# microsoft/ptgnn

Measured on NVIDIA H100. Metric: edges/sec per GNN layer, higher is better.
Workload: dtype f32

## Files before the change

### ptgnn_b200/csrc/plan.cu

```cuda
#include "common.cuh"

namespace ptgnn {

constexpr int SCAN_THREADS = 256;
constexpr int SCAN_ITEMS = 16;
constexpr int SCAN_CHUNK = SCAN_THREADS * SCAN_ITEMS;

__device__ __forceinline__ int warp_inclusive_scan(int v) {
    const int lane = threadIdx.x & 31;
#pragma unroll
    for (int o = 1; o < 32; o <<= 1) {
        int n = __shfl_up_sync(0xffffffffu, v, o);
        if (lane >= o) v += n;
    }
    return v;
}

template <int THREADS>
__device__ __forceinline__ int block_exclusive_scan(int v, int *total) {
    __shared__ int warp_sums[THREADS / 32];
    __shared__ int block_total;
    const int lane = threadIdx.x & 31, warp = threadIdx.x >> 5;
    int incl = warp_inclusive_scan(v);
    if (lane == 31) warp_sums[warp] = incl;
// ... 157 lines not shown
        }
    }
    __syncthreads();
#pragma unroll
    for (int r = 0; r < SORT_ROUNDS; ++r) {
        const bool valid = digit[r] < RADIX;
        const unsigned peers = __match_any_sync(0xffffffffu, digit[r]);
        int dst = 0;
        if (valid) dst = warp_hist[warp][digit[r]] + __popc(peers & ((1u << lane) - 1u));
        __syncwarp();
        if (valid && lane == __ffs(peers) - 1) warp_hist[warp][digit[r]] += __popc(peers);
        __syncwarp();
        if (valid) {
            keys_out[dst] = key[r];
            vals_out[dst] = val[r];
        }
    }
}

__global__ void __launch_bounds__(256) finalize_plan_kernel(const __grid_constant__ TypeOffsets toff, int64_t num_edges,
                                                            const int32_t *__restrict__ perm,
                                                            const int32_t *__restrict__ src32,
                                                            int32_t *__restrict__ pos, int32_t *__restrict__ src_sorted,
                                                            uint8_t *__restrict__ etype_sorted) {
    for (int64_t j = (int64_t)blockIdx.x * blockDim.x + threadIdx.x; j < num_edges;
         j += (int64_t)gridDim.x * blockDim.x) {
        const int32_t e = perm[j];
        pos[e] = (int32_t)j;
        src_sorted[j] = src32[e];
        etype_sorted[j] = (uint8_t)type_of_edge(toff.off, toff.num_types, e);
    }
}

struct PlanWs {
    size_t deg, scan_sums, keys_a, keys_b, vals_a, vals_b, hist, hist_sums, total;
};
static PlanWs plan_ws_layout(int64_t N, int64_t E) {
    PlanWs w{};
    const int64_t nblk = ceil_div(E > 0 ? E : 1, SORT_CHUNK);
    size_t o = 0;
    auto add = [&](size_t cnt) { size_t at = o; o += ws_slice(cnt, 4); return at; };
    w.deg = add((size_t)N + 1);
    w.scan_sums = add(scan_workspace_elems(N + 1));
    w.keys_a = add((size_t)E + 1);
    w.keys_b = add((size_t)E + 1);
    w.vals_a = add((size_t)E + 1);
    w.vals_b = add((size_t)E + 1);
    w.hist = add((size_t)RADIX * nblk);
    w.hist_sums = add(scan_workspace_elems((int64_t)RADIX * nblk));
    w.total = o;
    return w;
}

static int sort_edges_by_key(const int32_t *keys_in, int key_bits, int64_t E, int32_t *perm, char *ws, const PlanWs &L,
                             cudaStream_t st, const int32_t **sorted_keys = nullptr) {
    const int64_t nblk = ceil_div(E, SORT_CHUNK);
    int32_t *keys[2] = {reinterpret_cast<int32_t *>(ws + L.keys_a), reinterpret_cast<int32_t *>(ws + L.keys_b)};
    int32_t *vals[2] = {reinterpret_cast<int32_t *>(ws + L.vals_a), reinterpret_cast<int32_t *>(ws + L.vals_b)};
    int32_t *hist = reinterpret_cast<int32_t *>(ws + L.hist);
    int32_t *hist_sums = reinterpret_cast<int32_t *>(ws + L.hist_sums);
    const int passes = (key_bits + RADIX_BITS - 1) / RADIX_BITS;
    const int32_t *kin = keys_in;
    const int32_t *vin = nullptr;
    for (int p = 0; p < passes; ++p) {
        int32_t *kout = keys[p & 1];
        int32_t *vout = (p == passes - 1) ? perm : vals[p & 1];
        {
            TimedScope timed__(PTGNN_KERNEL_PLAN, st);
            radix_hist_kernel<<<(unsigned)nblk, SORT_THREADS, 0, st>>>(kin, E, p * RADIX_BITS, hist);
        }
        PTGNN_LAUNCHED();
        int rc = exclusive_scan_i32(hist, hist, (int64_t)RADIX * nblk, hist_sums, nullptr, st);
        if (rc) return rc;
        {
            TimedScope timed__(PTGNN_KERNEL_PLAN, st);
            radix_scatter_kernel<<<(unsigned)nblk, SORT_THREADS, 0, st>>>(kin, vin, E, p * RADIX_BITS, p == 0, hist, kout,
                                                                      vout);
        }
        PTGNN_LAUNCHED();
        kin = kout;
        vin = vout;
    }
    if (sorted_keys) *sorted_keys = kin;
    return PTGNN_OK;
}
static int bits_for(int64_t n) {
    int bits = 1;
    while (bits < 31 && ((int64_t)1 << bits) < n) ++bits;
    return bits;
}
static int sort_edges_by_target(const int32_t *tgt32, int64_t N, int64_t E, int32_t *perm, char *ws, const PlanWs &L,
                                cudaStream_t st) {
    return sort_edges_by_key(tgt32, bits_for(N), E, perm, ws, L, st);
}

__global__ void __launch_bounds__(256) block_keys_kernel(const __grid_constant__ TypeOffsets toff, int64_t num_edges,
                                                         const int32_t *__restrict__ tgt32, int B, int32_t *__restrict__ keys,
                                                         int32_t *__restrict__ group_count) {
    for (int64_t e = (int64_t)blockIdx.x * blockDim.x + threadIdx.x; e < num_edges; e += (int64_t)gridDim.x * blockDim.x) {
        const int t = type_of_edge(toff.off, toff.num_types, e);
        const int v = tgt32[e];
        const int blk = v / B, tl = v - blk * B;
        keys[e] = (blk * toff.num_types + t) * B + tl;
        atomicAdd(&group_count[(int64_t)blk * toff.num_types + t], 1);
    }
}
__global__ void __launch_bounds__(256) block_finalize_kernel(int64_t num_edges, int B, const int32_t *__restrict__ perm,
                                                             const int32_t *__restrict__ sorted_keys,
                                                             const int32_t *__restrict__ src32, int32_t *__restrict__ src_f,
                                                             uint8_t *__restrict__ tl_f) {
    for (int64_t j = (int64_t)blockIdx.x * blockDim.x + threadIdx.x; j < num_edges; j += (int64_t)gridDim.x * blockDim.x) {
        src_f[j] = src32[perm[j]];
        tl_f[j] = (uint8_t)(sorted_keys[j] % B);
    }
}
struct BlockPlanWs { size_t keys, perm, scan_sums, plan, total; };
static BlockPlanWs block_plan_ws_layout(int64_t N, int64_t E, int T, int B) {
    BlockPlanWs w{};
    const int64_t nblk = ceil_div(N > 0 ? N : 1, B), groups = nblk * (T > 0 ? T : 1) + 1;
    size_t o = 0;
    auto add = [&](size_t cnt) { size_t at = o; o += ws_slice(cnt, 4); return at; };
    w.keys = add((size_t)E + 1);
    w.perm = add((size_t)E + 1);
    w.scan_sums = add(scan_workspace_elems(groups));
    w.plan = o; o += plan_ws_layout(N, E).total;
    w.total = o;
    return w;
}

}

using namespace ptgnn;

extern "C" size_t ptgnn_b200_plan_workspace_bytes(int64_t num_nodes, int64_t num_edges) {
    if (num_nodes < 0 || num_edges < 0) return 0;
    return plan_ws_layout(num_nodes, num_edges).total;
}

static int plan_build_phases(int phases, int64_t num_nodes, int64_t num_source_nodes, int32_t num_types,
                             const int64_t *const *src_ptrs, const int64_t *const *tgt_ptrs, const int64_t *counts, int32_t *row_ptr,
                             int32_t *perm, int32_t *pos, int32_t *src_sorted, uint8_t *etype_sorted, int32_t *src32, int32_t *tgt32,
                             int32_t *status, void *workspace, size_t workspace_bytes, void *stream) {
    cudaStream_t st = static_cast<cudaStream_t>(stream);
    PTGNN_CHECK_ARG(num_nodes >= 0 && num_nodes < INT32_MAX, "plan_build: num_nodes=%lld out of range", (long long)num_nodes);
    if (num_source_nodes <= 0) num_source_nodes = num_nodes;
    PTGNN_CHECK_ARG(num_source_nodes < INT32_MAX, "plan_build: num_source_nodes out of range");
    PTGNN_CHECK_ARG(num_types >= 0 && num_types <= PTGNN_MAX_EDGE_TYPES, "plan_build: num_types=%d (max %d)", num_types,
                    PTGNN_MAX_EDGE_TYPES);
    PTGNN_CHECK_ARG(row_ptr && status, "plan_build: null row_ptr/status");
    EdgeTables tabs{};
    TypeOffsets toff{};
    tabs.num_types = toff.num_types = num_types;
    int64_t E = 0;
    for (int t = 0; t < num_types; ++t) {
        PTGNN_CHECK_ARG(counts[t] >= 0, "plan_build: negative edge count for type %d", t);
        PTGNN_CHECK_ARG(counts[t] == 0 || !(phases & 1) || (src_ptrs[t] && tgt_ptrs[t]), "plan_build: null edge list for type %d", t);
        tabs.src[t] = (phases & 1) ? src_ptrs[t] : nullptr;
        tabs.tgt[t] = (phases & 1) ? tgt_ptrs[t] : nullptr;
        tabs.off[t] = E;
        toff.off[t] = (int32_t)E;
        E += counts[t];
        PTGNN_CHECK_ARG(E < INT32_MAX, "plan_build: more than 2^31-1 edges");
    }
    tabs.off[num_types] = E;
    toff.off[num_types] = (int32_t)E;
    for (int t = num_types + 1; t <= PTGNN_MAX_EDGE_TYPES; ++t) { tabs.off[t] = E; toff.off[t] = (int32_t)E; }

    const PlanWs L = plan_ws_layout(num_nodes, E);
    PTGNN_CHECK_WORKSPACE("plan_build", workspace, workspace_bytes, L.total);
    char *ws = static_cast<char *>(workspace);
    int32_t *deg = reinterpret_cast<int32_t *>(ws + L.deg);

    const unsigned grid = (unsigned)(ceil_div(E > 0 ? E : 1, 256) < 132 * 16 ? ceil_div(E > 0 ? E : 1, 256) : 132 * 16);
    int rc = PTGNN_OK;
    if (phases & 1) {
        PTGNN_CUDA(cudaMemsetAsync(status, 0, sizeof(int32_t), st));
        PTGNN_CUDA(cudaMemsetAsync(deg, 0, sizeof(int32_t) * (size_t)(num_nodes + 1), st));
        if (E == 0) {
// ... 14 lines not shown
    PTGNN_CHECK_ARG(perm && pos && src_sorted && etype_sorted && src32 && tgt32, "plan_build: null output array");
    rc = sort_edges_by_target(tgt32, num_nodes, E, perm, ws, L, st);
    if (rc) return rc;
    {
        TimedScope timed__(PTGNN_KERNEL_PLAN, st);
        finalize_plan_kernel<<<grid, 256, 0, st>>>(toff, E, perm, src32, pos, src_sorted, etype_sorted);
    }
    PTGNN_LAUNCHED();
    return PTGNN_OK;
}

extern "C" int ptgnn_b200_plan_build(int64_t num_nodes, int64_t num_source_nodes, int32_t num_types,
                                     const int64_t *const *src_ptrs, const int64_t *const *tgt_ptrs, const int64_t *counts,
                                     int32_t *row_ptr, int32_t *perm, int32_t *pos, int32_t *src_sorted, uint8_t *etype_sorted,
                                     int32_t *src32, int32_t *tgt32, int32_t *status, void *workspace, size_t workspace_bytes,
                                     void *stream) {
    return plan_build_phases(3, num_nodes, num_source_nodes, num_types, src_ptrs, tgt_ptrs, counts, row_ptr, perm, pos, src_sorted,
                             etype_sorted, src32, tgt32, status, workspace, workspace_bytes, stream);
}
extern "C" int ptgnn_b200_plan_convert(int64_t num_nodes, int64_t num_source_nodes, int32_t num_types,
                                       const int64_t *const *src_ptrs, const int64_t *const *tgt_ptrs, const int64_t *counts,
                                       int32_t *row_ptr, int32_t *src32, int32_t *tgt32, int32_t *status, void *workspace,
                                       size_t workspace_bytes, void *stream) {
    return plan_build_phases(1, num_nodes, num_source_nodes, num_types, src_ptrs, tgt_ptrs, counts, row_ptr, nullptr, nullptr, nullptr,
                             nullptr, src32, tgt32, status, workspace, workspace_bytes, stream);
}
extern "C" int ptgnn_b200_plan_sort(int64_t num_nodes, int32_t num_types, const int64_t *counts, int32_t *perm, int32_t *pos,
                                    int32_t *src_sorted, uint8_t *etype_sorted, const int32_t *src32, const int32_t *tgt32,
                                    void *workspace, size_t workspace_bytes, void *stream) {
    int32_t dummy_status = 0;
    return plan_build_phases(2, num_nodes, num_nodes, num_types, nullptr, nullptr, counts, &dummy_status , perm, pos,
                             src_sorted, etype_sorted, const_cast<int32_t *>(src32), const_cast<int32_t *>(tgt32), &dummy_status, workspace,
                             workspace_bytes, stream);
}

extern "C" size_t ptgnn_b200_block_plan_workspace_bytes(int64_t num_nodes, int64_t num_edges, int32_t num_types,
                                                        int32_t block_targets) {
    if (num_nodes < 0 || num_edges < 0 || num_types < 0 || block_targets <= 0) return 0;
    return block_plan_ws_layout(num_nodes, num_edges, num_types, block_targets).total;
}

extern "C" int ptgnn_b200_block_plan_build(int64_t num_nodes, int32_t num_types, const int64_t *type_off,
                                           const int32_t *src32, const int32_t *tgt32, int32_t block_targets,
                                           int32_t *group_off, int32_t *src_f, uint8_t *tl_f, void *workspace,
                                           size_t workspace_bytes, void *stream) {
    cudaStream_t st = static_cast<cudaStream_t>(stream);
    const int B = block_targets, T = num_types;
    PTGNN_CHECK_ARG(num_nodes >= 0 && num_nodes < INT32_MAX, "block_plan_build: num_nodes out of range");
    PTGNN_CHECK_ARG(T > 0 && T <= PTGNN_MAX_EDGE_TYPES && type_off, "block_plan_build: bad num_types=%d", T);
    PTGNN_CHECK_ARG(B >= 8 && B <= 256, "block_plan_build: block_targets=%d must be in [8, 256]", B);
    const int64_t E = type_off[T];
    PTGNN_CHECK_ARG(E >= 0 && E < INT32_MAX, "block_plan_build: edge count out of range");
    const int64_t nblk = ceil_div(num_nodes, B), groups = nblk * T;
    PTGNN_CHECK_ARG(nblk * T * B < ((int64_t)1 << 31), "block_plan_build: %lld blocks x %d types x %d targets overflow the 31-bit sort key",
                    (long long)nblk, T, B);
    PTGNN_CHECK_ARG(group_off, "block_plan_build: null group_off");
    const BlockPlanWs L = block_plan_ws_layout(num_nodes, E, T, B);
    PTGNN_CHECK_WORKSPACE("block_plan_build", workspace, workspace_bytes, L.total);
    PTGNN_CUDA(cudaMemsetAsync(group_off, 0, sizeof(int32_t) * (size_t)(groups + 1), st));
    if (E == 0 || num_nodes == 0) return PTGNN_OK;
    PTGNN_CHECK_ARG(src32 && tgt32 && src_f && tl_f, "block_plan_build: null edge array");
    char *ws = static_cast<char *>(workspace);
    int32_t *keys = reinterpret_cast<int32_t *>(ws + L.keys), *perm = reinterpret_cast<int32_t *>(ws + L.perm);
    TypeOffsets toff{};
    toff.num_types = T;
    for (int t = 0; t <= PTGNN_MAX_EDGE_TYPES; ++t) toff.off[t] = (int32_t)type_off[t < T ? t : T];
    const unsigned grid = (unsigned)(ceil_div(E, 256) < 132 * 16 ? ceil_div(E, 256) : 132 * 16);
    {
        TimedScope timed__(PTGNN_KERNEL_PLAN, st);
        block_keys_kernel<<<grid, 256, 0, st>>>(toff, E, tgt32, B, keys, group_off);
    }
    PTGNN_LAUNCHED();
    int rc = exclusive_scan_i32(group_off, group_off, groups + 1, reinterpret_cast<int32_t *>(ws + L.scan_sums), nullptr, st);
    if (rc) return rc;
    const int32_t *sorted_keys = nullptr;
    rc = sort_edges_by_key(keys, bits_for(nblk * T * B), E, perm, ws + L.plan, plan_ws_layout(num_nodes, E), st, &sorted_keys);
    if (rc) return rc;
    {
        TimedScope timed__(PTGNN_KERNEL_PLAN, st);
        block_finalize_kernel<<<grid, 256, 0, st>>>(E, B, perm, sorted_keys, src32, src_f, tl_f);
    }
    PTGNN_LAUNCHED();
    return PTGNN_OK;
}
```

### ptgnn_b200/csrc/fused_mp.cu

```cuda
#include "fused_mp.cuh"

#include <cuda_bf16.h>
#include <cuda_fp16.h>
#include <float.h>
#include <stdlib.h>

#include <type_traits>

#include "tc_common.cuh"

namespace ptgnn {
namespace fused {

using tc::mbar_arrive;
using tc::mbar_init;
using tc::mbar_wait;

constexpr int NUM_THREADS = 16 * 32;
constexpr int GATHER_WARP0 = 8, GATHER_THREADS = 64;
constexpr int SCHED_WARP = 10;
constexpr int REDUCER_WARP0 = 12;
constexpr int SCHED_READER_WARPS = 8 + 2 + 4;
constexpr int NUM_SLOTS = 3, LOOKAHEAD = 2;
constexpr int SLOT_BYTES = 32768;
constexpr int RING_BYTES = NUM_SLOTS * SLOT_BYTES;
constexpr int META_RING = 8;
constexpr int SCHED_RING = 4;
constexpr int PRODUCER_REGS = 56, CONSUMER_REGS = 184, REDUCER_REGS = 88;
static_assert(PRODUCER_REGS + 2 * CONSUMER_REGS + REDUCER_REGS <= 4 * 128, "register budgets exceed the launch allocation");
constexpr int NMAX = 64;
constexpr int ACC_PITCH = NMAX + 4;
constexpr int ACC_BYTES = kD * ACC_PITCH * 4;
constexpr int RED_BAR_ID = 1;

struct Meta {
    int32_t tloff[128];
    uint32_t endmask[4];
    int32_t n, pad[3];
};
struct Sched {
    int32_t blk, pad[3];
    int32_t off[PTGNN_MAX_EDGE_TYPES + 4];
};
constexpr int ACC_OFF = RING_BYTES;
constexpr int AGG_OFF = RING_BYTES + ACC_BYTES;
__host__ __device__ constexpr int agg_bytes(int B) { return B * kD * 4; }
constexpr int SMEM_TAIL = META_RING * (int)sizeof(Meta) + SCHED_RING * (int)sizeof(Sched) + 256 ;
constexpr int smem_bytes(int B) { return 1024 + RING_BYTES + ACC_BYTES + agg_bytes(B) + SMEM_TAIL; }
static_assert(smem_bytes(kMaxBlockTargets) <= 232448, "shared memory budget");

struct Params {
    const unsigned char *src_rows, *tgt_rows;
    const uint4 *wpack;
    const int32_t *group_off, *src_f;
    const uint8_t *tl_f;
    const int32_t *row_ptr;
    void *out;
    int num_nodes, num_blocks, B, T, reduce, out_mode;
    int32_t *status;
    unsigned long long *trace;
    Epilogue epi;
    EgcEpilogue egc;
};
constexpr int EPI_AGG = 0, EPI_EGC = 1;

__device__ __forceinline__ uint4 ldg_nc_u4(const uint4 *p) {
    uint4 r;
    asm volatile("ld.global.nc.L1::no_allocate.v4.u32 {%0,%1,%2,%3}, [%4];" : "=r"(r.x), "=r"(r.y), "=r"(r.z), "=r"(r.w) : "l"(p));
    return r;
}
__device__ __forceinline__ void named_bar_sync(int id, int threads) { asm volatile("bar.sync %0, %1;" ::"r"(id), "r"(threads) : "memory"); }
__device__ __forceinline__ uint32_t swz(int row, int q) { return (uint32_t)(row * 128 + ((q ^ (row & 7)) << 4)); }

constexpr int TRACE_ROLES = 4, TRACE_CAP = 8192;
__shared__ uint32_t trace_n[TRACE_ROLES];
__device__ __forceinline__ void trace_mark(const Params &p, int tag, uint32_t step) {
    if (p.trace == nullptr || blockIdx.x != 0) return;
    const int tid = (int)threadIdx.x;
    const int role = tid == GATHER_WARP0 * 32 ? 0 : (tid == 0 ? 1 : (tid == 128 ? 2 : (tid == REDUCER_WARP0 * 32 ? 3 : -1)));
    if (role < 0) return;
    const uint32_t n = trace_n[role];
    if (n >= TRACE_CAP) return;
    p.trace[role * TRACE_CAP + n] = ((unsigned long long)clock64() << 24) | ((unsigned long long)(step & 0xFFFFu) << 8) | (unsigned)(tag & 0xFF);
    trace_n[role] = n + 1;
}

struct Step { int blk, t, e, n, seg; };
template <int NSEG>
struct StepGen {
    const Sched *sched;
    uint64_t *sfull, *sempty;
    int T, nmax, lane;
    uint32_t it = 0;
    const Sched *tab = nullptr;
    int blk = -1, t = 0, e = 0, e1 = 0, seg = 0;
    __device__ __forceinline__ int next(Step &s) {
        for (;;) {
            if (tab == nullptr) {
                const uint32_t r = it % SCHED_RING;
                mbar_wait(&sfull[r], (it / SCHED_RING) & 1);
                blk = sched[r].blk;
                if (blk < 0) return 2;
                tab = &sched[r];
                t = -1; e = e1 = 0; seg = 0;
            }
            if (e < e1) {
                s.blk = blk; s.t = t; s.e = e; s.n = min(nmax, e1 - e); s.seg = seg;
                if (++seg == NSEG) { seg = 0; e += nmax; }
                return 0;
            }
            ++t;
            while (t < T && tab->off[t + 1] == tab->off[t]) ++t;
            if (t >= T) {
                tab = nullptr;
                s.blk = blk;
                __syncwarp();
                if (lane == 0) mbar_arrive(&sempty[it % SCHED_RING]);
                ++it;
                return 1;
            }
            e = tab->off[t]; e1 = tab->off[t + 1]; seg = 0;
        }
    }
// ... 363 lines not shown
                    if (lane == 0) m->endmask[c >> 5] = word;
                }
                if (g == 0) m->n = st.n;
                ++sgc;
            };
            auto issue_next = [&]() {
                cur = nxt;
                int idx[NMAX / 8];
#pragma unroll
                for (int i = 0; i < NMAX / 8; ++i) idx[i] = idx_nxt[i];
                finish_meta(cur);
                const uint32_t slot = c_issue % NUM_SLOTS;
                trace_mark(p, 1, c_issue);
                mbar_wait(&x_empty[slot], ((c_issue / NUM_SLOTS) & 1) ^ 1);
                trace_mark(p, 2, c_issue);
                const unsigned char *rows = cur.seg == 0 ? p.src_rows : p.tgt_rows;
                const uint32_t sbase = smem_u32(ring + slot * SLOT_BYTES) + swz(rsub, q);
#pragma unroll
                for (int i = 0; i < NMAX / 8; ++i) {
                    if (idx[i] >= 0) {
                        const unsigned char *src = rows + (size_t)idx[i] * ROW_BYTES + q * 16;
#pragma unroll
                        for (int ti = 0; ti < NT; ++ti)
                            cp_async16(sbase + ti * TILE_BYTES + i * 1024, src + (ti / KCH) * (K * 2) + (ti % KCH) * 128, 16);
                    }
                }
                trace_mark(p, 3, c_issue);
                ++c_issue;
            };
            fetch();
            bool more = has_nxt;
            while (more) {
                const uint32_t slot = c_issue % NUM_SLOTS;
                issue_next();
                asm volatile("cp.async.mbarrier.arrive.noinc.shared::cta.b64 [%0];" ::"r"(smem_u32(&x_full[slot])) : "memory");
                trace_mark(p, 4, c_done);
                mbar_arrive(&x_full[slot]);
                ++c_done;
                fetch();
                more = has_nxt;
            }
            cp_async_wait<0>();
        }
    } else {
        tc::reg_alloc<CONSUMER_REGS>();
        const int eg = warp >> 2, ew = warp & 3;
        const int gq = lane >> 2, tq = lane & 3;
        const int f0 = 64 * eg + 16 * ew + gq;
        StepGen<NSEG> gen{sched, sched_full, sched_empty, T, NMAX, lane};
        uint32_t sg = 0, xs = 0;
        int w_t = -1, w_seg = -1;
        uint32_t wf[NPART][K / 16][4];
        float acc_m[32], acc_c[32];
        auto load_weights = [&](const Step &st) {
            const uint32_t *wp = reinterpret_cast<const uint32_t *>(p.wpack + (size_t)(st.t * NSEG + st.seg) * NPART * (K / 8) * 128);
#pragma unroll
            for (int part = 0; part < NPART; ++part)
#pragma unroll
                for (int ks = 0; ks < K / 16; ++ks)
#pragma unroll
                    for (int i = 0; i < 4; ++i) {
                        const int c4 = (part * (K / 8) + 2 * ks + (i >> 1)), f = f0 + 8 * (i & 1);
                        wf[part][ks][i] = __ldg(wp + ((size_t)c4 * 128 + f) * 4 + tq);
                    }
            w_t = st.t; w_seg = st.seg;
            trace_mark(p, 11, xs);
        };
        auto mma = [&](auto nb_tag, uint32_t slot_addr) {
            constexpr int NB = decltype(nb_tag)::value;
#pragma unroll
            for (int ks = 0; ks < K / 16; ++ks) {
                const int kc = ks >> 2, kk = ks & 3;
                const uint64_t x_hi = tc::make_smem_desc_sw128(slot_addr + kc * TILE_BYTES) + kk * 2;
                const uint64_t x_lo = tc::make_smem_desc_sw128(slot_addr + (KCH + kc) * TILE_BYTES) + kk * 2;
                auto one = [&](float (&dacc)[32], const uint32_t (&a)[4], uint64_t desc) {
                    if (NB == 1) tc::wgmma_16_rs_n16<BF16>(dacc, a, desc);
                    else if (NB == 2) tc::wgmma_16_rs_n32<BF16>(dacc, a, desc);
                    else if (NB == 3) tc::wgmma_16_rs_n48<BF16>(dacc, a, desc);
                    else tc::wgmma_16_rs_n64<BF16>(dacc, a, desc);
                };
                one(acc_m, wf[0][ks], x_hi);
                if (NPROD == 3) {
                    one(acc_c, wf[0][ks], x_lo);
                    one(acc_c, wf[NPART - 1][ks], x_hi);
                }
            }
        };
        Step s, nx;
        int ev = gen.next(s);
        while (ev != 2) {
            if (ev == 0) {
                trace_mark(p, 10, xs);
                if (s.t != w_t || s.seg != w_seg) load_weights(s);
                const uint32_t slot = xs % NUM_SLOTS;
                mbar_wait(&x_full[slot], (xs / NUM_SLOTS) & 1);
                tc::fence_proxy_async_smem();
                trace_mark(p, 12, xs);
                if (tc::warp_uniform(s.seg) == 0) {
#pragma unroll
                    for (int i = 0; i < 32; ++i) { acc_m[i] = 0.0f; acc_c[i] = 0.0f; }
                }
                const uint32_t slot_addr = smem_u32(ring + slot * SLOT_BYTES);
                const int nb = tc::warp_uniform((s.n + 15) >> 4);
                tc::wgmma_fence();
                using std::integral_constant;
                if (nb == 1) mma(integral_constant<int, 1>{}, slot_addr);
                else if (nb == 2) mma(integral_constant<int, 2>{}, slot_addr);
                else if (nb == 3) mma(integral_constant<int, 3>{}, slot_addr);
                else mma(integral_constant<int, 4>{}, slot_addr);
                tc::wgmma_commit();
                trace_mark(p, 13, xs);
                tc::wgmma_wait<0>();
                tc::fence_acc(acc_m);
                if (NPROD == 3) tc::fence_acc(acc_c);
                __syncwarp();
                if (lane == 0) mbar_arrive(&x_empty[slot]);
                trace_mark(p, 14, xs);
                ++xs;
                const int evn = gen.next(nx);
                if (evn == 0 && (nx.t != w_t || nx.seg != w_seg)) load_weights(nx);
                if (s.seg == NSEG - 1) {
                    trace_mark(p, 20, sg);
                    mbar_wait(acc_empty, (sg & 1) ^ 1);
                    trace_mark(p, 21, sg);
#pragma unroll
                    for (int j = 0; j < 8; ++j) {
                        if (8 * j < 16 * nb) {
#pragma unroll
                        for (int h = 0; h < 2; ++h) {
                            float v0 = acc_m[4 * j + 2 * h], v1 = acc_m[4 * j + 2 * h + 1];
                            if (NPROD == 3) {
                                v0 = fmaf(acc_c[4 * j + 2 * h], 1.0f / 2048.0f, v0); v1 = fmaf(acc_c[4 * j + 2 * h + 1], 1.0f / 2048.0f, v1);
                            } else {
                                v0 = __bfloat162float(__float2bfloat16_rn(v0)); v1 = __bfloat162float(__float2bfloat16_rn(v1));
                            }
                            *reinterpret_cast<float2 *>(acc_s + (f0 + 8 * h) * ACC_PITCH + 8 * j + 2 * tq) = make_float2(v0, v1);
                        }
                        }
                    }
                    __syncwarp();
                    if (lane == 0) mbar_arrive(acc_full);
                    trace_mark(p, 22, sg);
                    ++sg;
                }
                s = nx; ev = evn;
                continue;
            }
            ev = gen.next(s);
        }
    }
}

__global__ void __launch_bounds__(256) pack_states_kernel(const float *__restrict__ h, long long rows, int K,
                                                          uint4 *__restrict__ out, int32_t *__restrict__ status) {
    const long long total = rows * (K / 8);
    bool bad = false;
    for (long long i = (long long)blockIdx.x * blockDim.x + threadIdx.x; i < total; i += (long long)gridDim.x * blockDim.x) {
        const long long row = i / (K / 8);
        const int c8 = (int)(i - row * (K / 8));
        const float4 a = ld_stream_f4(reinterpret_cast<const float4 *>(h + row * K + c8 * 8));
        const float4 b = ld_stream_f4(reinterpret_cast<const float4 *>(h + row * K + c8 * 8 + 4));
        const float x[8] = {a.x, a.y, a.z, a.w, b.x, b.y, b.z, b.w};
        __half hi[8], lo[8];
#pragma unroll
        for (int j = 0; j < 8; ++j) bad |= !split_f16(x[j], hi[j], lo[j]);
        uint4 vh, vl;
        vh.x = pack_h2(hi[0], hi[1]); vh.y = pack_h2(hi[2], hi[3]); vh.z = pack_h2(hi[4], hi[5]); vh.w = pack_h2(hi[6], hi[7]);
        vl.x = pack_h2(lo[0], lo[1]); vl.y = pack_h2(lo[2], lo[3]); vl.z = pack_h2(lo[4], lo[5]); vl.w = pack_h2(lo[6], lo[7]);
        uint4 *dst = out + row * (K / 4);
        dst[c8] = vh;
        dst[K / 8 + c8] = vl;
    }
    if (bad && status != nullptr) *reinterpret_cast<volatile int32_t *>(status) = 1;
}

struct WeightSrc {
    const float *w[PTGNN_MAX_EDGE_TYPES];
};
template <int NPROD>
__global__ void __launch_bounds__(256) pack_weights_kernel(const __grid_constant__ WeightSrc src, int num_types, int K, int nseg,
                                                           RowMap rows, uint4 *__restrict__ out, int32_t *__restrict__ status) {
    constexpr int NPART = NPROD == 3 ? 2 : 1;
    const int per_mat = nseg * (K / 8) * 128;
    const long long total = (long long)num_types * per_mat;
    bool bad = false;
    for (long long i = (long long)blockIdx.x * blockDim.x + threadIdx.x; i < total; i += (long long)gridDim.x * blockDim.x) {
        const int t = (int)(i / per_mat);
        int r = (int)(i - (long long)t * per_mat);
        const int seg = r / ((K / 8) * 128);
        r -= seg * (K / 8) * 128;
        const int c4 = r / 128, d = r % 128;
        int srow = d;
        if (rows.bases > 0) {
            const int o = rows.col0 + d / rows.bases, b = d % rows.bases;
            srow = ((o / rows.dh) * rows.bases + b) * rows.dh + o % rows.dh;
        }
        const float *row = src.w[t] + (size_t)srow * (nseg * K) + seg * K + c4 * 8;
        float x[8];
#pragma unroll
        for (int j = 0; j < 8; ++j) x[j] = row[j];
        const size_t base = ((size_t)(t * nseg + seg) * NPART) * (K / 8) * 128;
        if (NPROD == 3) {
            __half hi[8], lo[8];
#pragma unroll
            for (int j = 0; j < 8; ++j) bad |= !split_f16(x[j], hi[j], lo[j]);
            uint4 vh, vl;
            vh.x = pack_h2(hi[0], hi[1]); vh.y = pack_h2(hi[2], hi[3]); vh.z = pack_h2(hi[4], hi[5]); vh.w = pack_h2(hi[6], hi[7]);
            vl.x = pack_h2(lo[0], lo[1]); vl.y = pack_h2(lo[2], lo[3]); vl.z = pack_h2(lo[4], lo[5]); vl.w = pack_h2(lo[6], lo[7]);
            out[base + (size_t)c4 * 128 + d] = vh;
            out[base + (size_t)(K / 8 + c4) * 128 + d] = vl;
        } else {
            uint4 v;
            __nv_bfloat162 p0 = __floats2bfloat162_rn(x[0], x[1]), p1 = __floats2bfloat162_rn(x[2], x[3]);
            __nv_bfloat162 p2 = __floats2bfloat162_rn(x[4], x[5]), p3 = __floats2bfloat162_rn(x[6], x[7]);
            v.x = *reinterpret_cast<uint32_t *>(&p0); v.y = *reinterpret_cast<uint32_t *>(&p1);
            v.z = *reinterpret_cast<uint32_t *>(&p2); v.w = *reinterpret_cast<uint32_t *>(&p3);
            out[base + (size_t)c4 * 128 + d] = v;
        }
    }
    if (bad && status != nullptr) *reinterpret_cast<volatile int32_t *>(status + 1) = 1;
}

bool supported(int nprod, int K, int D, int use_target) {
    (void)use_target;
    if (D != kD) return false;
    if (nprod == 3) return K == 64 || K == 128;
    if (nprod == 1) return K == 64 || K == 128 || K == 256;
    return false;
}
size_t packed_weight_bytes(int nprod, int num_types, int K, int use_target) {
    const int nseg = use_target ? 2 : 1, npart = nprod == 3 ? 2 : 1;
    return ws_slice((size_t)num_types * nseg * npart * (K / 8) * 128, 16);
}
size_t packed_state_bytes(int nprod, int64_t rows, int K) {
    return nprod == 3 ? ws_slice((size_t)rows * K * 4 + 16, 1) : 0;
}
int recommended_block_targets(int64_t num_nodes) {
    if (num_nodes <= 0) return kMaxBlockTargets;
    const int64_t waves = ceil_div(num_nodes, (int64_t)kMaxBlockTargets * 132);
    int64_t B = ceil_div(num_nodes, waves * 132);
    B = (B + 7) / 8 * 8;
    if (B < 8) B = 8;
    if (B > kMaxBlockTargets) B = kMaxBlockTargets;
    return (int)B;
}

int pack_weights(int nprod, int num_types, int K, int use_target, const float *const *weights, void *packed, int32_t *status,
                 cudaStream_t st, RowMap rows) {
    WeightSrc src{};
    for (int t = 0; t < num_types; ++t) src.w[t] = weights[t];
    const int nseg = use_target ? 2 : 1;
    {
        TimedScope timed__(PTGNN_KERNEL_PACK, st);
        if (nprod == 3) pack_weights_kernel<3><<<132, 256, 0, st>>>(src, num_types, K, nseg, rows, static_cast<uint4 *>(packed), status);
        else pack_weights_kernel<1><<<132, 256, 0, st>>>(src, num_types, K, nseg, rows, static_cast<uint4 *>(packed), status);
    }
    PTGNN_LAUNCHED();
    return PTGNN_OK;
}

int pack_states(const float *h, int64_t rows, int K, void *packed, int32_t *status, cudaStream_t st) {
    if (rows <= 0) return PTGNN_OK;
    const int64_t items = rows * (K / 8);
    const unsigned grid = (unsigned)(ceil_div(items, 256) < 132 * 8 ? ceil_div(items, 256) : 132 * 8);
    {
        TimedScope timed__(PTGNN_KERNEL_PACK, st);
        pack_states_kernel<<<grid, 256, 0, st>>>(h, (long long)rows, K, static_cast<uint4 *>(packed), status);
    }
    PTGNN_LAUNCHED();
    return PTGNN_OK;
}

template <int NPROD, int K, int NSEG, int RED, int EPI = EPI_AGG>
static int launch_one(const Params &p, cudaStream_t st) {
    auto kernel = fused_aggregate_kernel<NPROD, K, NSEG, RED, EPI>;
    const int smem = smem_bytes(p.B);
    PTGNN_CUDA(cudaFuncSetAttribute(kernel, cudaFuncAttributeMaxDynamicSharedMemorySize, smem));
    const int sms = sm_count();
    const int grid = p.num_blocks < sms ? p.num_blocks : sms;
    {
        TimedScope timed__(PTGNN_KERNEL_MESSAGE, st);
        kernel<<<grid, NUM_THREADS, smem, st>>>(p);
    }
    PTGNN_LAUNCHED();
    return PTGNN_OK;
// ... 80 lines not shown
```

Before: 1.339 billion.

## Replace global radix sort in block plan with bucket scatter and per-group sort

The block plan build no longer runs a multi-pass global radix sort over composite keys. Instead it counts edges per (block, type) group using warp-aggregated atomics, scans the counts, and scatters packed (target-local, edge-id) items into group buckets. Each bucket is then sorted in place: small groups by a per-warp rank sort in shared memory, large ones by a CTA-wide radix sort. This cuts the number of full-array passes and launches, at the cost of nondeterministic scatter order fixed by the per-group sort, and quadratic work for groups near the size cap.

Result: faster. 1.372 billion (median of 6 runs) (+2.4%).

```diff
diff --git a/ptgnn_b200/csrc/plan.cu b/ptgnn_b200/csrc/plan.cu
--- a/ptgnn_b200/csrc/plan.cu
+++ b/ptgnn_b200/csrc/plan.cu
@@ -233,15 +233,20 @@
     return w;
 }
 
-static int sort_edges_by_key(const int32_t *keys_in, int key_bits, int64_t E, int32_t *perm, char *ws, const PlanWs &L,
-                             cudaStream_t st, const int32_t **sorted_keys = nullptr) {
+static int bits_for(int64_t n) {
+    int bits = 1;
+    while (bits < 31 && ((int64_t)1 << bits) < n) ++bits;
+    return bits;
+}
+static int sort_edges_by_target(const int32_t *tgt32, int64_t N, int64_t E, int32_t *perm, char *ws, const PlanWs &L,
+                                cudaStream_t st) {
     const int64_t nblk = ceil_div(E, SORT_CHUNK);
     int32_t *keys[2] = {reinterpret_cast<int32_t *>(ws + L.keys_a), reinterpret_cast<int32_t *>(ws + L.keys_b)};
     int32_t *vals[2] = {reinterpret_cast<int32_t *>(ws + L.vals_a), reinterpret_cast<int32_t *>(ws + L.vals_b)};
     int32_t *hist = reinterpret_cast<int32_t *>(ws + L.hist);
     int32_t *hist_sums = reinterpret_cast<int32_t *>(ws + L.hist_sums);
-    const int passes = (key_bits + RADIX_BITS - 1) / RADIX_BITS;
-    const int32_t *kin = keys_in;
+    const int passes = (bits_for(N) + RADIX_BITS - 1) / RADIX_BITS;
+    const int32_t *kin = tgt32;
     const int32_t *vin = nullptr;
     for (int p = 0; p < passes; ++p) {
         int32_t *kout = keys[p & 1];
@@ -262,49 +267,173 @@
         kin = kout;
         vin = vout;
     }
-    if (sorted_keys) *sorted_keys = kin;
     return PTGNN_OK;
 }
-static int bits_for(int64_t n) {
-    int bits = 1;
-    while (bits < 31 && ((int64_t)1 << bits) < n) ++bits;
-    return bits;
-}
-static int sort_edges_by_target(const int32_t *tgt32, int64_t N, int64_t E, int32_t *perm, char *ws, const PlanWs &L,
-                                cudaStream_t st) {
-    return sort_edges_by_key(tgt32, bits_for(N), E, perm, ws, L, st);
-}
-
-__global__ void __launch_bounds__(256) block_keys_kernel(const __grid_constant__ TypeOffsets toff, int64_t num_edges,
-                                                         const int32_t *__restrict__ tgt32, int B, int32_t *__restrict__ keys,
-                                                         int32_t *__restrict__ group_count) {
+
+struct EdgeGroup { int64_t g; int tl; };
+__device__ __forceinline__ EdgeGroup edge_group(const TypeOffsets &toff, const int32_t *__restrict__ tgt32, int B, int64_t e) {
+    const int t = type_of_edge(toff.off, toff.num_types, e);
+    const int v = tgt32[e];
+    const int blk = v / B;
+    return {(int64_t)blk * toff.num_types + t, v - blk * B};
+}
+
+__global__ void __launch_bounds__(256) block_count_kernel(const __grid_constant__ TypeOffsets toff, int64_t num_edges,
+                                                          const int32_t *__restrict__ tgt32, int B, int32_t *__restrict__ group_count) {
     for (int64_t e = (int64_t)blockIdx.x * blockDim.x + threadIdx.x; e < num_edges; e += (int64_t)gridDim.x * blockDim.x) {
-        const int t = type_of_edge(toff.off, toff.num_types, e);
-        const int v = tgt32[e];
-        const int blk = v / B, tl = v - blk * B;
-        keys[e] = (blk * toff.num_types + t) * B + tl;
-        atomicAdd(&group_count[(int64_t)blk * toff.num_types + t], 1);
-    }
-}
-__global__ void __launch_bounds__(256) block_finalize_kernel(int64_t num_edges, int B, const int32_t *__restrict__ perm,
-                                                             const int32_t *__restrict__ sorted_keys,
-                                                             const int32_t *__restrict__ src32, int32_t *__restrict__ src_f,
-                                                             uint8_t *__restrict__ tl_f) {
-    for (int64_t j = (int64_t)blockIdx.x * blockDim.x + threadIdx.x; j < num_edges; j += (int64_t)gridDim.x * blockDim.x) {
-        src_f[j] = src32[perm[j]];
-        tl_f[j] = (uint8_t)(sorted_keys[j] % B);
-    }
-}
-struct BlockPlanWs { size_t keys, perm, scan_sums, plan, total; };
+        const int64_t g = edge_group(toff, tgt32, B, e).g;
+        const unsigned peers = __match_any_sync(__activemask(), (unsigned long long)g);
+        if ((threadIdx.x & 31) == __ffs(peers) - 1) atomicAdd(&group_count[g], __popc(peers));
+    }
+}
+
+__global__ void __launch_bounds__(256) block_scatter_kernel(const __grid_constant__ TypeOffsets toff, int64_t num_edges,
+                                                            const int32_t *__restrict__ tgt32, int B,
+                                                            const int32_t *__restrict__ group_off, int32_t *__restrict__ group_count,
+                                                            uint64_t *__restrict__ items) {
+    for (int64_t e = (int64_t)blockIdx.x * blockDim.x + threadIdx.x; e < num_edges; e += (int64_t)gridDim.x * blockDim.x) {
+        const EdgeGroup eg = edge_group(toff, tgt32, B, e);
+        const int lane = threadIdx.x & 31;
+        const unsigned peers = __match_any_sync(__activemask(), (unsigned long long)eg.g);
+        const int leader = __ffs(peers) - 1;
+        int left = 0;
+        if (lane == leader) left = atomicSub(&group_count[eg.g], __popc(peers));
+        left = __shfl_sync(peers, left, leader);
+        const int32_t slot = group_off[eg.g] + left - 1 - __popc(peers & ((1u << lane) - 1u));
+        items[slot] = ((uint64_t)eg.tl << 32) | (uint32_t)e;
+    }
+}
+
+constexpr int GSORT_WARPS = 8;
+constexpr int GSORT_THREADS = GSORT_WARPS * 32;
+constexpr int GSORT_CAP = 512;
+constexpr int GSORT_ILP = 2;
+constexpr int GSORT_RADIX_PASSES = 5;
+
+struct GroupSortSmem {
+    union {
+        uint64_t warp_items[GSORT_WARPS][GSORT_CAP];
+        struct {
+            int bin[256];
+            int warp_cnt[GSORT_WARPS][256];
+        } radix;
+    };
+};
+
+__device__ __forceinline__ void write_group(uint64_t it, int64_t j, const int32_t *__restrict__ src32, int32_t *__restrict__ src_f,
+                                            uint8_t *__restrict__ tl_f) {
+    src_f[j] = src32[(uint32_t)it];
+    tl_f[j] = (uint8_t)(it >> 32);
+}
+
+__device__ __noinline__ void cta_radix_sort_group(GroupSortSmem &sm, uint64_t *__restrict__ items, uint64_t *__restrict__ items_alt, int64_t lo,
+                                     int n, const int32_t *__restrict__ src32, int32_t *__restrict__ src_f, uint8_t *__restrict__ tl_f) {
+    const int tid = threadIdx.x, lane = tid & 31, warp = tid >> 5;
+    const uint64_t *in = items + lo;
+    uint64_t *out = items_alt + lo;
+    for (int p = 0; p < GSORT_RADIX_PASSES; ++p) {
+        const int shift = 8 * p;
+        sm.radix.bin[tid] = 0;
+        __syncthreads();
+        for (int i = tid; i < n; i += GSORT_THREADS) atomicAdd(&sm.radix.bin[(in[i] >> shift) & 255], 1);
+        __syncthreads();
+        int total;
+        sm.radix.bin[tid] = block_exclusive_scan<GSORT_THREADS>(sm.radix.bin[tid], &total);
+        for (int64_t base = 0; base < n; base += GSORT_THREADS) {
+#pragma unroll
+            for (int w = 0; w < GSORT_WARPS; ++w) sm.radix.warp_cnt[w][tid] = 0;
+            __syncthreads();
+            const int64_t i = base + tid;
+            const bool valid = i < n;
+            const uint64_t it = valid ? in[i] : 0;
+            const int d = valid ? (int)((it >> shift) & 255) : 256;
+            const unsigned peers = __match_any_sync(0xffffffffu, d);
+            const int rank = __popc(peers & ((1u << lane) - 1u));
+            if (valid && lane == __ffs(peers) - 1) sm.radix.warp_cnt[warp][d] = __popc(peers);
+            __syncthreads();
+            {
+                int run = sm.radix.bin[tid];
+#pragma unroll
+                for (int w = 0; w < GSORT_WARPS; ++w) {
+                    const int c = sm.radix.warp_cnt[w][tid];
+                    sm.radix.warp_cnt[w][tid] = run;
+                    run += c;
+                }
+                sm.radix.bin[tid] = run;
+            }
+            __syncthreads();
+            if (valid) out[sm.radix.warp_cnt[warp][d] + rank] = it;
+            __syncthreads();
+        }
+        const uint64_t *next_in = out;
+        out = const_cast<uint64_t *>(in);
+        in = next_in;
+    }
+    for (int i = tid; i < n; i += GSORT_THREADS) write_group(in[i], lo + i, src32, src_f, tl_f);
+    __syncthreads();
+}
+
+__global__ void __launch_bounds__(GSORT_THREADS) block_group_sort_kernel(int64_t groups, const int32_t *__restrict__ group_off,
+                                                                         uint64_t *__restrict__ items, uint64_t *__restrict__ items_alt,
+                                                                         const int32_t *__restrict__ src32, int32_t *__restrict__ src_f,
+                                                                         uint8_t *__restrict__ tl_f) {
+    __shared__ GroupSortSmem sm;
+    const int lane = threadIdx.x & 31, warp = threadIdx.x >> 5;
+    const int64_t g0 = (int64_t)blockIdx.x * GSORT_WARPS;
+    if (g0 + warp < groups) {
+        const int64_t lo = group_off[g0 + warp];
+        const int n = group_off[g0 + warp + 1] - (int32_t)lo;
+        if (n <= GSORT_CAP) {
+            uint64_t *s = sm.warp_items[warp];
+            for (int base = 0; base < n; base += 32 * GSORT_ILP) {
+                uint64_t v[GSORT_ILP];
+#pragma unroll
+                for (int q = 0; q < GSORT_ILP; ++q) v[q] = base + q * 32 + lane < n ? items[lo + base + q * 32 + lane] : 0;
+#pragma unroll
+                for (int q = 0; q < GSORT_ILP; ++q)
+                    if (base + q * 32 + lane < n) s[base + q * 32 + lane] = v[q];
+            }
+            __syncwarp();
+            for (int base = 0; base < n; base += 32 * GSORT_ILP) {
+                uint64_t mine[GSORT_ILP];
+                int rank[GSORT_ILP];
+#pragma unroll
+                for (int q = 0; q < GSORT_ILP; ++q) {
+                    mine[q] = base + q * 32 + lane < n ? s[base + q * 32 + lane] : 0;
+                    rank[q] = 0;
+                }
+#pragma unroll 4
+                for (int j = 0; j < n; ++j) {
+                    const uint64_t x = s[j];
+#pragma unroll
+                    for (int q = 0; q < GSORT_ILP; ++q) rank[q] += x < mine[q];
+                }
+#pragma unroll
+                for (int q = 0; q < GSORT_ILP; ++q)
+                    if (base + q * 32 + lane < n) write_group(mine[q], lo + rank[q], src32, src_f, tl_f);
+            }
+        }
+    }
+    for (int w = 0; w < GSORT_WARPS && g0 + w < groups; ++w) {
+        const int64_t lo = group_off[g0 + w];
+        const int n = group_off[g0 + w + 1] - (int32_t)lo;
+        if (n > GSORT_CAP) {
+            __syncthreads();
+            cta_radix_sort_group(sm, items, items_alt, lo, n, src32, src_f, tl_f);
+        }
+    }
+}
+
+struct BlockPlanWs { size_t group_count, scan_sums, items, items_alt, total; };
 static BlockPlanWs block_plan_ws_layout(int64_t N, int64_t E, int T, int B) {
     BlockPlanWs w{};
     const int64_t nblk = ceil_div(N > 0 ? N : 1, B), groups = nblk * (T > 0 ? T : 1) + 1;
     size_t o = 0;
-    auto add = [&](size_t cnt) { size_t at = o; o += ws_slice(cnt, 4); return at; };
-    w.keys = add((size_t)E + 1);
-    w.perm = add((size_t)E + 1);
-    w.scan_sums = add(scan_workspace_elems(groups));
-    w.plan = o; o += plan_ws_layout(N, E).total;
+    auto add = [&](size_t cnt, size_t elt) { size_t at = o; o += ws_slice(cnt, elt); return at; };
+    w.group_count = add((size_t)groups, 4);
+    w.scan_sums = add(scan_workspace_elems(groups), 4);
+    w.items = add((size_t)E + 1, 8);
+    w.items_alt = add((size_t)E + 1, 8);
     w.total = o;
     return w;
 }
@@ -425,33 +554,40 @@
     const int64_t E = type_off[T];
     PTGNN_CHECK_ARG(E >= 0 && E < INT32_MAX, "block_plan_build: edge count out of range");
     const int64_t nblk = ceil_div(num_nodes, B), groups = nblk * T;
-    PTGNN_CHECK_ARG(nblk * T * B < ((int64_t)1 << 31), "block_plan_build: %lld blocks x %d types x %d targets overflow the 31-bit sort key",
+    PTGNN_CHECK_ARG(nblk * T * B < ((int64_t)1 << 31), "block_plan_build: %lld blocks x %d types x %d targets exceed 2^31",
                     (long long)nblk, T, B);
     PTGNN_CHECK_ARG(group_off, "block_plan_build: null group_off");
     const BlockPlanWs L = block_plan_ws_layout(num_nodes, E, T, B);
     PTGNN_CHECK_WORKSPACE("block_plan_build", workspace, workspace_bytes, L.total);
-    PTGNN_CUDA(cudaMemsetAsync(group_off, 0, sizeof(int32_t) * (size_t)(groups + 1), st));
-    if (E == 0 || num_nodes == 0) return PTGNN_OK;
+    if (E == 0 || num_nodes == 0) {
+        PTGNN_CUDA(cudaMemsetAsync(group_off, 0, sizeof(int32_t) * (size_t)(groups + 1), st));
+        return PTGNN_OK;
+    }
     PTGNN_CHECK_ARG(src32 && tgt32 && src_f && tl_f, "block_plan_build: null edge array");
     char *ws = static_cast<char *>(workspace);
-    int32_t *keys = reinterpret_cast<int32_t *>(ws + L.keys), *perm = reinterpret_cast<int32_t *>(ws + L.perm);
+    int32_t *group_count = reinterpret_cast<int32_t *>(ws + L.group_count);
+    uint64_t *items = reinterpret_cast<uint64_t *>(ws + L.items), *items_alt = reinterpret_cast<uint64_t *>(ws + L.items_alt);
     TypeOffsets toff{};
     toff.num_types = T;
     for (int t = 0; t <= PTGNN_MAX_EDGE_TYPES; ++t) toff.off[t] = (int32_t)type_off[t < T ? t : T];
     const unsigned grid = (unsigned)(ceil_div(E, 256) < 132 * 16 ? ceil_div(E, 256) : 132 * 16);
-    {
-        TimedScope timed__(PTGNN_KERNEL_PLAN, st);
-        block_keys_kernel<<<grid, 256, 0, st>>>(toff, E, tgt32, B, keys, group_off);
-    }
-    PTGNN_LAUNCHED();
-    int rc = exclusive_scan_i32(group_off, group_off, groups + 1, reinterpret_cast<int32_t *>(ws + L.scan_sums), nullptr, st);
+    PTGNN_CUDA(cudaMemsetAsync(group_count, 0, sizeof(int32_t) * (size_t)(groups + 1), st));
+    {
+        TimedScope timed__(PTGNN_KERNEL_PLAN, st);
+        block_count_kernel<<<grid, 256, 0, st>>>(toff, E, tgt32, B, group_count);
+    }
+    PTGNN_LAUNCHED();
+    int rc = exclusive_scan_i32(group_count, group_off, groups + 1, reinterpret_cast<int32_t *>(ws + L.scan_sums), nullptr, st);
     if (rc) return rc;
-    const int32_t *sorted_keys = nullptr;
-    rc = sort_edges_by_key(keys, bits_for(nblk * T * B), E, perm, ws + L.plan, plan_ws_layout(num_nodes, E), st, &sorted_keys);
-    if (rc) return rc;
-    {
-        TimedScope timed__(PTGNN_KERNEL_PLAN, st);
-        block_finalize_kernel<<<grid, 256, 0, st>>>(E, B, perm, sorted_keys, src32, src_f, tl_f);
+    {
+        TimedScope timed__(PTGNN_KERNEL_PLAN, st);
+        block_scatter_kernel<<<grid, 256, 0, st>>>(toff, E, tgt32, B, group_off, group_count, items);
+    }
+    PTGNN_LAUNCHED();
+    {
+        TimedScope timed__(PTGNN_KERNEL_PLAN, st);
+        block_group_sort_kernel<<<(unsigned)ceil_div(groups, GSORT_WARPS), GSORT_THREADS, 0, st>>>(groups, group_off, items, items_alt,
+                                                                                                  src32, src_f, tl_f);
     }
     PTGNN_LAUNCHED();
     return PTGNN_OK;
```

## Pack weights in per-lane fragment order and stagger reloads across warpgroups

Applied to the files above, without the earlier changes.

The weight packing kernel now writes the A-operand register fragments so that each consumer lane fetches one contiguous uint4 per k-step. This replaces four strided 32-bit loads per k-step with a single coalesced 16-byte load. Weight reloads are also split by warpgroup: the first reloads before the accumulator epilogue and the second after it, so their reload traffic does not overlap. This makes the packed layout and the device-side fragment mapping depend on each other, so any mismatch between them would give wrong results.

New measurement: 1.334 billion before, 1.372 billion after (median of 6 runs). 2.8% higher.

```diff
diff --git a/ptgnn_b200/csrc/fused_mp.cu b/ptgnn_b200/csrc/fused_mp.cu
--- a/ptgnn_b200/csrc/fused_mp.cu
+++ b/ptgnn_b200/csrc/fused_mp.cu
@@ -64,11 +64,6 @@
 };
 constexpr int EPI_AGG = 0, EPI_EGC = 1;
 
-__device__ __forceinline__ uint4 ldg_nc_u4(const uint4 *p) {
-    uint4 r;
-    asm volatile("ld.global.nc.L1::no_allocate.v4.u32 {%0,%1,%2,%3}, [%4];" : "=r"(r.x), "=r"(r.y), "=r"(r.z), "=r"(r.w) : "l"(p));
-    return r;
-}
 __device__ __forceinline__ void named_bar_sync(int id, int threads) { asm volatile("bar.sync %0, %1;" ::"r"(id), "r"(threads) : "memory"); }
 __device__ __forceinline__ uint32_t swz(int row, int q) { return (uint32_t)(row * 128 + ((q ^ (row & 7)) << 4)); }
 
@@ -539,16 +534,14 @@
         uint32_t wf[NPART][K / 16][4];
         float acc_m[32], acc_c[32];
         auto load_weights = [&](const Step &st) {
-            const uint32_t *wp = reinterpret_cast<const uint32_t *>(p.wpack + (size_t)(st.t * NSEG + st.seg) * NPART * (K / 8) * 128);
+            const uint4 *wp = p.wpack + (size_t)(st.t * NSEG + st.seg) * NPART * (K / 16) * 256 + warp * 32 + lane;
 #pragma unroll
             for (int part = 0; part < NPART; ++part)
 #pragma unroll
-                for (int ks = 0; ks < K / 16; ++ks)
-#pragma unroll
-                    for (int i = 0; i < 4; ++i) {
-                        const int c4 = (part * (K / 8) + 2 * ks + (i >> 1)), f = f0 + 8 * (i & 1);
-                        wf[part][ks][i] = __ldg(wp + ((size_t)c4 * 128 + f) * 4 + tq);
-                    }
+                for (int ks = 0; ks < K / 16; ++ks) {
+                    const uint4 v = __ldg(wp + (part * (K / 16) + ks) * 256);
+                    wf[part][ks][0] = v.x; wf[part][ks][1] = v.y; wf[part][ks][2] = v.z; wf[part][ks][3] = v.w;
+                }
             w_t = st.t; w_seg = st.seg;
             trace_mark(p, 11, xs);
         };
@@ -604,7 +597,9 @@
                 trace_mark(p, 14, xs);
                 ++xs;
                 const int evn = gen.next(nx);
-                if (evn == 0 && (nx.t != w_t || nx.seg != w_seg)) load_weights(nx);
+                const bool reload = evn == 0 && (nx.t != w_t || nx.seg != w_seg);
+                const bool reload_early = tc::warp_uniform(eg) == 0;
+                if (reload && reload_early) load_weights(nx);
                 if (s.seg == NSEG - 1) {
                     trace_mark(p, 20, sg);
                     mbar_wait(acc_empty, (sg & 1) ^ 1);
@@ -629,6 +624,7 @@
                     trace_mark(p, 22, sg);
                     ++sg;
                 }
+                if (reload && !reload_early) load_weights(nx);
                 s = nx; ev = evn;
                 continue;
             }
@@ -667,25 +663,29 @@
 __global__ void __launch_bounds__(256) pack_weights_kernel(const __grid_constant__ WeightSrc src, int num_types, int K, int nseg,
                                                            RowMap rows, uint4 *__restrict__ out, int32_t *__restrict__ status) {
     constexpr int NPART = NPROD == 3 ? 2 : 1;
-    const int per_mat = nseg * (K / 8) * 128;
-    const long long total = (long long)num_types * per_mat;
+    const int per_seg = (K / 16) * 256;
+    const long long total = (long long)num_types * nseg * per_seg;
     bool bad = false;
     for (long long i = (long long)blockIdx.x * blockDim.x + threadIdx.x; i < total; i += (long long)gridDim.x * blockDim.x) {
-        const int t = (int)(i / per_mat);
-        int r = (int)(i - (long long)t * per_mat);
-        const int seg = r / ((K / 8) * 128);
-        r -= seg * (K / 8) * 128;
-        const int c4 = r / 128, d = r % 128;
-        int srow = d;
-        if (rows.bases > 0) {
-            const int o = rows.col0 + d / rows.bases, b = d % rows.bases;
-            srow = ((o / rows.dh) * rows.bases + b) * rows.dh + o % rows.dh;
-        }
-        const float *row = src.w[t] + (size_t)srow * (nseg * K) + seg * K + c4 * 8;
+        const int ts = (int)(i / per_seg);
+        const int r = (int)(i - (long long)ts * per_seg);
+        const int t = ts / nseg, seg = ts - t * nseg;
+        const int ks = r / 256, c = r % 256;
+        const int f = 16 * (c >> 5) + ((c & 31) >> 2), tq = c & 3;
         float x[8];
 #pragma unroll
-        for (int j = 0; j < 8; ++j) x[j] = row[j];
-        const size_t base = ((size_t)(t * nseg + seg) * NPART) * (K / 8) * 128;
+        for (int j = 0; j < 4; ++j) {
+            const int d = f + 8 * (j & 1);
+            int srow = d;
+            if (rows.bases > 0) {
+                const int o = rows.col0 + d / rows.bases, b = d % rows.bases;
+                srow = ((o / rows.dh) * rows.bases + b) * rows.dh + o % rows.dh;
+            }
+            const float *row = src.w[t] + (size_t)srow * (nseg * K) + seg * K + 16 * ks + 8 * (j >> 1) + 2 * tq;
+            x[2 * j] = row[0];
+            x[2 * j + 1] = row[1];
+        }
+        const size_t base = (size_t)ts * NPART * per_seg + r;
         if (NPROD == 3) {
             __half hi[8], lo[8];
 #pragma unroll
@@ -693,15 +693,15 @@
             uint4 vh, vl;
             vh.x = pack_h2(hi[0], hi[1]); vh.y = pack_h2(hi[2], hi[3]); vh.z = pack_h2(hi[4], hi[5]); vh.w = pack_h2(hi[6], hi[7]);
             vl.x = pack_h2(lo[0], lo[1]); vl.y = pack_h2(lo[2], lo[3]); vl.z = pack_h2(lo[4], lo[5]); vl.w = pack_h2(lo[6], lo[7]);
-            out[base + (size_t)c4 * 128 + d] = vh;
-            out[base + (size_t)(K / 8 + c4) * 128 + d] = vl;
+            out[base] = vh;
+            out[base + per_seg] = vl;
         } else {
             uint4 v;
             __nv_bfloat162 p0 = __floats2bfloat162_rn(x[0], x[1]), p1 = __floats2bfloat162_rn(x[2], x[3]);
             __nv_bfloat162 p2 = __floats2bfloat162_rn(x[4], x[5]), p3 = __floats2bfloat162_rn(x[6], x[7]);
             v.x = *reinterpret_cast<uint32_t *>(&p0); v.y = *reinterpret_cast<uint32_t *>(&p1);
             v.z = *reinterpret_cast<uint32_t *>(&p2); v.w = *reinterpret_cast<uint32_t *>(&p3);
-            out[base + (size_t)c4 * 128 + d] = v;
+            out[base] = v;
         }
     }
     if (bad && status != nullptr) *reinterpret_cast<volatile int32_t *>(status + 1) = 1;
@@ -716,7 +716,7 @@
 }
 size_t packed_weight_bytes(int nprod, int num_types, int K, int use_target) {
     const int nseg = use_target ? 2 : 1, npart = nprod == 3 ? 2 : 1;
-    return ws_slice((size_t)num_types * nseg * npart * (K / 8) * 128, 16);
+    return ws_slice((size_t)num_types * nseg * npart * (K / 16) * 256, 16);
 }
 size_t packed_state_bytes(int nprod, int64_t rows, int K) {
     return nprod == 3 ? ws_slice((size_t)rows * K * 4 + 16, 1) : 0;
```

## Pack weights in wgmma fragment order and split weight prefetch across steps

Applied to the files above, without the earlier changes.

The weight packing kernel now writes weights directly in per-warp, per-lane register-fragment order, so each consumer thread loads a whole k-step fragment with one 16-byte load instead of four scattered 4-byte loads. The prefetch of the next step's weights is split: the first half of the k-steps is loaded right after the current MMA, and the remaining half just before the next MMA. The aim is fewer, better-coalesced global loads and less register pressure or latency exposure during weight switches. The cost is an extra flag and a more involved packing index computation.

Result: faster. 1.347 billion before, 1.380 billion after, median of 6 (+2.5%).

```diff
diff --git a/ptgnn_b200/csrc/fused_mp.cu b/ptgnn_b200/csrc/fused_mp.cu
--- a/ptgnn_b200/csrc/fused_mp.cu
+++ b/ptgnn_b200/csrc/fused_mp.cu
@@ -538,20 +538,26 @@
         int w_t = -1, w_seg = -1;
         uint32_t wf[NPART][K / 16][4];
         float acc_m[32], acc_c[32];
-        auto load_weights = [&](const Step &st) {
-            const uint32_t *wp = reinterpret_cast<const uint32_t *>(p.wpack + (size_t)(st.t * NSEG + st.seg) * NPART * (K / 8) * 128);
+        auto load_weights = [&](const Step &st, auto ks0_tag, auto ks1_tag) {
+            constexpr int KS0 = decltype(ks0_tag)::value, KS1 = decltype(ks1_tag)::value;
+            const uint4 *wp = p.wpack + (size_t)(st.t * NSEG + st.seg) * NPART * (K / 16) * 256 + 32 * warp + lane;
 #pragma unroll
             for (int part = 0; part < NPART; ++part)
 #pragma unroll
-                for (int ks = 0; ks < K / 16; ++ks)
-#pragma unroll
-                    for (int i = 0; i < 4; ++i) {
-                        const int c4 = (part * (K / 8) + 2 * ks + (i >> 1)), f = f0 + 8 * (i & 1);
-                        wf[part][ks][i] = __ldg(wp + ((size_t)c4 * 128 + f) * 4 + tq);
-                    }
-            w_t = st.t; w_seg = st.seg;
-            trace_mark(p, 11, xs);
+                for (int ks = KS0; ks < KS1; ++ks) {
+                    const uint4 v = __ldg(wp + (part * (K / 16) + ks) * 256);
+                    wf[part][ks][0] = v.x; wf[part][ks][1] = v.y; wf[part][ks][2] = v.z; wf[part][ks][3] = v.w;
+                }
+            if (KS0 == 0) {
+                w_t = st.t; w_seg = st.seg;
+                trace_mark(p, 11, xs);
+            }
         };
+        using std::integral_constant;
+        constexpr integral_constant<int, 0> KS_FIRST{};
+        constexpr integral_constant<int, K / 32> KS_SPLIT{};
+        constexpr integral_constant<int, K / 16> KS_END{};
+        bool w_tail = false;
         auto mma = [&](auto nb_tag, uint32_t slot_addr) {
             constexpr int NB = decltype(nb_tag)::value;
 #pragma unroll
@@ -577,7 +583,9 @@
         while (ev != 2) {
             if (ev == 0) {
                 trace_mark(p, 10, xs);
-                if (s.t != w_t || s.seg != w_seg) load_weights(s);
+                if (s.t != w_t || s.seg != w_seg) load_weights(s, KS_FIRST, KS_END);
+                else if (w_tail) load_weights(s, KS_SPLIT, KS_END);
+                w_tail = false;
                 const uint32_t slot = xs % NUM_SLOTS;
                 mbar_wait(&x_full[slot], (xs / NUM_SLOTS) & 1);
                 tc::fence_proxy_async_smem();
@@ -589,7 +597,6 @@
                 const uint32_t slot_addr = smem_u32(ring + slot * SLOT_BYTES);
                 const int nb = tc::warp_uniform((s.n + 15) >> 4);
                 tc::wgmma_fence();
-                using std::integral_constant;
                 if (nb == 1) mma(integral_constant<int, 1>{}, slot_addr);
                 else if (nb == 2) mma(integral_constant<int, 2>{}, slot_addr);
                 else if (nb == 3) mma(integral_constant<int, 3>{}, slot_addr);
@@ -604,7 +611,10 @@
                 trace_mark(p, 14, xs);
                 ++xs;
                 const int evn = gen.next(nx);
-                if (evn == 0 && (nx.t != w_t || nx.seg != w_seg)) load_weights(nx);
+                if (evn == 0 && (nx.t != w_t || nx.seg != w_seg)) {
+                    load_weights(nx, KS_FIRST, KS_SPLIT);
+                    w_tail = true;
+                }
                 if (s.seg == NSEG - 1) {
                     trace_mark(p, 20, sg);
                     mbar_wait(acc_empty, (sg & 1) ^ 1);
@@ -667,25 +677,33 @@
 __global__ void __launch_bounds__(256) pack_weights_kernel(const __grid_constant__ WeightSrc src, int num_types, int K, int nseg,
                                                            RowMap rows, uint4 *__restrict__ out, int32_t *__restrict__ status) {
     constexpr int NPART = NPROD == 3 ? 2 : 1;
-    const int per_mat = nseg * (K / 8) * 128;
+    const int per_mat = nseg * (K / 16) * 256;
     const long long total = (long long)num_types * per_mat;
     bool bad = false;
     for (long long i = (long long)blockIdx.x * blockDim.x + threadIdx.x; i < total; i += (long long)gridDim.x * blockDim.x) {
         const int t = (int)(i / per_mat);
         int r = (int)(i - (long long)t * per_mat);
-        const int seg = r / ((K / 8) * 128);
-        r -= seg * (K / 8) * 128;
-        const int c4 = r / 128, d = r % 128;
-        int srow = d;
-        if (rows.bases > 0) {
-            const int o = rows.col0 + d / rows.bases, b = d % rows.bases;
-            srow = ((o / rows.dh) * rows.bases + b) * rows.dh + o % rows.dh;
-        }
-        const float *row = src.w[t] + (size_t)srow * (nseg * K) + seg * K + c4 * 8;
+        const int seg = r / ((K / 16) * 256);
+        r -= seg * (K / 16) * 256;
+        const int ks = r / 256, u = r % 256;
+        const int f0 = 16 * (u >> 5) + ((u >> 2) & 7), c0 = 16 * ks + 2 * (u & 3);
         float x[8];
 #pragma unroll
-        for (int j = 0; j < 8; ++j) x[j] = row[j];
-        const size_t base = ((size_t)(t * nseg + seg) * NPART) * (K / 8) * 128;
+        for (int h = 0; h < 2; ++h) {
+            const int d = f0 + 8 * h;
+            int srow = d;
+            if (rows.bases > 0) {
+                const int o = rows.col0 + d / rows.bases, b = d % rows.bases;
+                srow = ((o / rows.dh) * rows.bases + b) * rows.dh + o % rows.dh;
+            }
+            const float *row = src.w[t] + (size_t)srow * (nseg * K) + seg * K + c0;
+#pragma unroll
+            for (int c8 = 0; c8 < 2; ++c8) {
+                x[2 * (2 * c8 + h)] = row[8 * c8];
+                x[2 * (2 * c8 + h) + 1] = row[8 * c8 + 1];
+            }
+        }
+        const size_t base = ((size_t)(t * nseg + seg) * NPART * (K / 16) + ks) * 256 + u;
         if (NPROD == 3) {
             __half hi[8], lo[8];
 #pragma unroll
@@ -693,15 +711,15 @@
             uint4 vh, vl;
             vh.x = pack_h2(hi[0], hi[1]); vh.y = pack_h2(hi[2], hi[3]); vh.z = pack_h2(hi[4], hi[5]); vh.w = pack_h2(hi[6], hi[7]);
             vl.x = pack_h2(lo[0], lo[1]); vl.y = pack_h2(lo[2], lo[3]); vl.z = pack_h2(lo[4], lo[5]); vl.w = pack_h2(lo[6], lo[7]);
-            out[base + (size_t)c4 * 128 + d] = vh;
-            out[base + (size_t)(K / 8 + c4) * 128 + d] = vl;
+            out[base] = vh;
+            out[base + (size_t)(K / 16) * 256] = vl;
         } else {
             uint4 v;
             __nv_bfloat162 p0 = __floats2bfloat162_rn(x[0], x[1]), p1 = __floats2bfloat162_rn(x[2], x[3]);
             __nv_bfloat162 p2 = __floats2bfloat162_rn(x[4], x[5]), p3 = __floats2bfloat162_rn(x[6], x[7]);
             v.x = *reinterpret_cast<uint32_t *>(&p0); v.y = *reinterpret_cast<uint32_t *>(&p1);
             v.z = *reinterpret_cast<uint32_t *>(&p2); v.w = *reinterpret_cast<uint32_t *>(&p3);
-            out[base + (size_t)c4 * 128 + d] = v;
+            out[base] = v;
         }
     }
     if (bad && status != nullptr) *reinterpret_cast<volatile int32_t *>(status + 1) = 1;
```
